# turbulencia/tlab

Measured on AMD Instinct MI355X. Metric: grid-point-updates/s per RK substep, higher is better.
Workload: dtype f64

## Files before the change

### tlab_amd/csrc/fftz.hip

```cpp
#include <hip/hip_runtime.h>

#include <cmath>
#include <cstdlib>
#include <stdexcept>
#include <string>
#include <vector>

#include "fftz.hpp"
#include "profile.hpp"

namespace tlab {

struct cd {
    double x, y;
};
__device__ __forceinline__ cd operator+(cd a, cd b) { return {a.x + b.x, a.y + b.y}; }
__device__ __forceinline__ cd operator-(cd a, cd b) { return {a.x - b.x, a.y - b.y}; }
__device__ __forceinline__ cd cmul(cd a, cd b) { return {a.x * b.x - a.y * b.y, a.x * b.y + a.y * b.x}; }
template <int SGN>
__device__ __forceinline__ cd mul_pm_i(cd a) {
    return SGN > 0 ? cd{-a.y, a.x} : cd{a.y, -a.x};
}

template <int SGN>
// ... 21 lines not shown
    v[1] = e1 + o1; v[5] = e1 - o1;
    v[2] = e2 + o2; v[6] = e2 - o2;
    v[3] = e3 + o3; v[7] = e3 - o3;
}

__device__ __forceinline__ int ilog2(int v) { return 31 - __builtin_clz(v); }

struct FftzArgs {
    const double2 *in;
    double2 *out;
    const double2 *tw;
    long long nlines;
    int n;
    int npass;
    int radix[8];
};

template <int R, int SGN, int T>
__device__ __forceinline__ void fftz_pass(const FftzArgs &a, int t, int j, int Ns, bool first, bool last, long long col, bool colok, cd *lds) {
    const int n = a.n, m = n / R;
    cd v[R];
    if (first) {
#pragma unroll
        for (int r = 0; r < R; ++r) {
            double2 w = make_double2(0.0, 0.0);
            if (colok) w = a.in[col + (long long)(j + r * m) * a.nlines];
            v[r] = {w.x, w.y};
        }
    } else {
#pragma unroll
        for (int r = 0; r < R; ++r) v[r] = lds[(j + r * m) * T + t];
    }
    const int lNs = ilog2(Ns), lR = ilog2(R), ln = ilog2(n);
    const int k0 = (j & (Ns - 1)) << (ln - lNs - lR);
#pragma unroll
    for (int r = 1; r < R; ++r) {
        const double2 w = a.tw[(k0 * r) & (n - 1)];
        v[r] = cmul(v[r], cd{w.x, SGN > 0 ? -w.y : w.y});
    }
    if (R == 8) dft8<SGN>(reinterpret_cast<cd(&)[8]>(v));
    else if (R == 4) dft4<SGN>(v[0], v[1 % R], v[2 % R], v[3 % R]);
    else dft2<SGN>(v[0], v[1 % R]);
    const int j0 = ((j >> lNs) << (lNs + lR)) + (j & (Ns - 1));
    if (!first) __syncthreads();
    if (last) {
        if (colok) {
#pragma unroll
            for (int r = 0; r < R; ++r) a.out[col + (long long)(j0 + r * Ns) * a.nlines] = make_double2(v[r].x, v[r].y);
        }
    } else {
#pragma unroll
        for (int r = 0; r < R; ++r) lds[(j0 + r * Ns) * T + t] = v[r];
        __syncthreads();
    }
}

template <int SGN, int T>
__global__ void __launch_bounds__(1024) k_fftz(FftzArgs a) {
    extern __shared__ double2 fz_lds[];
    cd *lds = reinterpret_cast<cd *>(fz_lds);
    const int t = threadIdx.x % T;
    const int jt = threadIdx.x / T;
    const long long col = (long long)blockIdx.x * T + t;
    const bool colok = col < a.nlines;
    int Ns = 1;
    for (int p = 0; p < a.npass; ++p) {
        const int R = a.radix[p];
        const bool first = p == 0, last = p == a.npass - 1;
        const int items = 8 / R;
        if (R == 8) {
            fftz_pass<8, SGN, T>(a, t, jt, Ns, first, last, col, colok, lds);
        } else {
            const int m8 = a.n / 8;
            if (R == 4) {
                cd keep[2][4];
                int j0s[2];
                for (int q = 0; q < 2; ++q) {
                    const int j = jt + q * m8, m = a.n / 4;
                    for (int r = 0; r < 4; ++r) {
                        if (first) {
                            double2 w = make_double2(0.0, 0.0);
                            if (colok) w = a.in[col + (long long)(j + r * m) * a.nlines];
                            keep[q][r] = {w.x, w.y};
                        } else {
                            keep[q][r] = lds[(j + r * m) * T + t];
                        }
                    }
                    const int k0 = (j & (Ns - 1)) * (a.n >> (ilog2(Ns) + 2));
                    for (int r = 1; r < 4; ++r) {
                        const double2 w = a.tw[(k0 * r) & (a.n - 1)];
                        keep[q][r] = cmul(keep[q][r], cd{w.x, SGN > 0 ? -w.y : w.y});
                    }
                    dft4<SGN>(keep[q][0], keep[q][1], keep[q][2], keep[q][3]);
                    j0s[q] = ((j >> ilog2(Ns)) << (ilog2(Ns) + 2)) + (j & (Ns - 1));
                }
                if (!first) __syncthreads();
                for (int q = 0; q < 2; ++q)
                    for (int r = 0; r < 4; ++r) {
                        if (last) {
                            if (colok) a.out[col + (long long)(j0s[q] + r * Ns) * a.nlines] = make_double2(keep[q][r].x, keep[q][r].y);
                        } else {
                            lds[(j0s[q] + r * Ns) * T + t] = keep[q][r];
                        }
                    }
                if (!last) __syncthreads();
            } else {
                cd keep[4][2];
                int j0s[4];
                for (int q = 0; q < 4; ++q) {
                    const int j = jt + q * m8, m = a.n / 2;
                    for (int r = 0; r < 2; ++r) {
                        if (first) {
                            double2 w = make_double2(0.0, 0.0);
                            if (colok) w = a.in[col + (long long)(j + r * m) * a.nlines];
                            keep[q][r] = {w.x, w.y};
                        } else {
                            keep[q][r] = lds[(j + r * m) * T + t];
                        }
                    }
                    const int k0 = (j & (Ns - 1)) * (a.n >> (ilog2(Ns) + 1));
                    const double2 w = a.tw[k0 & (a.n - 1)];
                    keep[q][1] = cmul(keep[q][1], cd{w.x, SGN > 0 ? -w.y : w.y});
                    dft2<SGN>(keep[q][0], keep[q][1]);
                    j0s[q] = ((j >> ilog2(Ns)) << (ilog2(Ns) + 1)) + (j & (Ns - 1));
                }
                if (!first) __syncthreads();
                for (int q = 0; q < 4; ++q)
                    for (int r = 0; r < 2; ++r) {
                        if (last) {
                            if (colok) a.out[col + (long long)(j0s[q] + r * Ns) * a.nlines] = make_double2(keep[q][r].x, keep[q][r].y);
                        } else {
                            lds[(j0s[q] + r * Ns) * T + t] = keep[q][r];
                        }
                    }
                if (!last) __syncthreads();
            }
            (void)items;
        }
        Ns *= R;
    }
}

struct FftxArgs {
    const double *in;
    double2 *out;
    const double2 *tw;
    long long nlines;
    int n, m;
    int npass;
    int radix[8];
    int tl, lines;
    const long long *kxoff;
    const int *kxw;
};

template <int R>
__device__ __forceinline__ void fftx_pass(const FftxArgs &a, const double2 *__restrict__ zin, bool ok, cd *lds, int jt, int Ns, bool first) {
    constexpr int Q = 8 / R;
    const int M = a.m, m = M / R;
    cd v[Q][R];
    int j0s[Q];
#pragma unroll
    for (int q = 0; q < Q; ++q) {
        const int j = jt + q * a.tl;
#pragma unroll
        for (int r = 0; r < R; ++r) {
            if (first) {
                double2 w = make_double2(0.0, 0.0);
// ... 59 lines not shown
        const cd B = {Zc.x, -Zc.y};
        const cd E = {0.5 * (A.x + B.x), 0.5 * (A.y + B.y)};
        const cd D = A - B;
        const cd O = {0.5 * D.y, -0.5 * D.x};
        const double2 w = a.tw[k];
        const cd T = cmul(cd{w.x, w.y}, O);
        out[k] = make_double2(E.x + T.x, E.y + T.y);
        if (k != M - k) out[M - k] = make_double2(E.x - T.x, -(E.y - T.y));
    }
}

struct FftxFinal {
    double *q, *h;
    double dte, kco;
    int scale, ny;
};

template <int R>
__device__ __forceinline__ void fftx_pass_inv(const FftxArgs &a, cd *lds, int jt, int Ns) {
    constexpr int Q = 8 / R;
    const int M = a.m, m = M / R;
    cd v[Q][R];
    int j0s[Q];
#pragma unroll
    for (int q = 0; q < Q; ++q) {
        const int j = jt + q * a.tl;
#pragma unroll
        for (int r = 0; r < R; ++r) v[q][r] = lds[j + r * m];
        const int k0 = (j & (Ns - 1)) << (ilog2(M) - ilog2(Ns) - ilog2(R));
#pragma unroll
// ... 2 lines not shown
            v[q][r] = cmul(v[q][r], cd{w.x, -w.y});
        }
        if (R == 8) dft8<+1>(reinterpret_cast<cd(&)[8]>(v[q]));
        else if (R == 4) dft4<+1>(v[q][0], v[q][1 % R], v[q][2 % R], v[q][3 % R]);
        else dft2<+1>(v[q][0], v[q][1 % R]);
        j0s[q] = ((j >> ilog2(Ns)) << (ilog2(Ns) + ilog2(R))) + (j & (Ns - 1));
    }
    __syncthreads();
#pragma unroll
    for (int q = 0; q < Q; ++q)
#pragma unroll
        for (int r = 0; r < R; ++r) lds[j0s[q] + r * Ns] = v[q][r];
    __syncthreads();
}

template <bool FINAL>
__global__ void __launch_bounds__(256) k_fftx_c2r(FftxArgs a, FftxFinal fin) {
    extern __shared__ double2 fx_lds[];
    const int jt = threadIdx.x & (a.tl - 1), ll = threadIdx.x >> ilog2(a.tl);
    const long long line = (long long)blockIdx.x * a.lines + ll;
    const bool ok = line < a.nlines;
    cd *lds = reinterpret_cast<cd *>(fx_lds) + (size_t)ll * a.m;
    const int M = a.m;
    if (ok) {
        const double2 *X = reinterpret_cast<const double2 *>(a.in) + line * (M + 1);
        const double2 *XP = reinterpret_cast<const double2 *>(a.in);
        for (int k = jt; k <= M / 2; k += a.tl) {
            double2 xa, xb;
            if (a.kxw != nullptr) { xa = XP[a.kxoff[k] + line * a.kxw[k]]; xb = XP[a.kxoff[M - k] + line * a.kxw[M - k]]; }
            else { xa = X[k]; xb = X[M - k]; }
            if (k == 0) { xa.y = 0.0; xb.y = 0.0; }
            const cd E = {xa.x + xb.x, xa.y - xb.y};
            const cd D = {xa.x - xb.x, xa.y + xb.y};
            const double2 w = a.tw[k];
            const cd O = cmul(D, cd{w.x, -w.y});
            if (k < M) lds[k % M] = {E.x - O.y, E.y + O.x};
            if (k != 0 && k != M - k) lds[M - k] = {E.x + O.y, -E.y + O.x};
        }
    }
    __syncthreads();
    int Ns = 1;
    for (int p = 0; p < a.npass; ++p) {
        const int R = a.radix[p];
        if (R == 8) fftx_pass_inv<8>(a, lds, jt, Ns);
        else if (R == 4) fftx_pass_inv<4>(a, lds, jt, Ns);
        else fftx_pass_inv<2>(a, lds, jt, Ns);
        Ns *= R;
    }
    if (!ok) return;
    if (!FINAL) {
        double2 *out = a.out + line * M;
        for (int j = jt; j < M; j += a.tl) out[j] = make_double2(lds[j].x, lds[j].y);
    } else {
        const int jy = a.nlines < (1LL << 31) ? (int)((unsigned)line % (unsigned)fin.ny) : (int)(line % fin.ny);
        const bool wall = jy == 0 || jy == fin.ny - 1;
        double2 *q2 = reinterpret_cast<double2 *>(fin.q) + line * M, *h2 = reinterpret_cast<double2 *>(fin.h) + line * M;
        for (int j = jt; j < M; j += a.tl) {
            const double2 hv0 = h2[j], qv = q2[j];
            double hx = hv0.x - lds[j].x, hy = hv0.y - lds[j].y;
            if (wall) { hx = 0.0; hy = 0.0; }
            q2[j] = make_double2(qv.x + fin.dte * hx, qv.y + fin.dte * hy);
            h2[j] = fin.scale ? make_double2(fin.kco * hx, fin.kco * hy) : make_double2(hx, hy);
        }
    }
}

bool FftxPlan::supported(int n) {
    if (n % 2 || n < 128 || n > 2048) return false;
    int m = n / 2;
    while (m % 8 == 0) m /= 8;
    return m == 1 || m == 2 || m == 4;
}

FftxPlan::FftxPlan(int n_, long long nlines_) : n(n_), nlines(nlines_) {
// ... 48 lines not shown
    const long double two_pi = 6.283185307179586476925286766559005768L;
    for (int k = 0; k < n; ++k) {
        tw[2 * k] = (double)cosl(two_pi * k / n);
        tw[2 * k + 1] = (double)(-sinl(two_pi * k / n));
    }
    if (hipMalloc((void **)&d_tw, tw.size() * sizeof(double)) != hipSuccess) throw std::runtime_error("FftzPlan: hipMalloc");
    if (hipMemcpy(d_tw, tw.data(), tw.size() * sizeof(double), hipMemcpyHostToDevice) != hipSuccess) throw std::runtime_error("FftzPlan: hipMemcpy");
}

FftzPlan::~FftzPlan() {
    if (d_tw) (void)hipFree(d_tw);
}

template <int T>
static void fftz_launch(int dir, const FftzArgs &a, hipStream_t st) {
    const unsigned grid = (unsigned)((a.nlines + T - 1) / T);
    const unsigned block = (unsigned)(T * a.n / 8);
    const size_t lds = (size_t)a.n * T * sizeof(double2);
    static bool attr_done = false;
    if (!attr_done) {
        (void)hipFuncSetAttribute(reinterpret_cast<const void *>(&k_fftz<-1, T>), hipFuncAttributeMaxDynamicSharedMemorySize, 160 * 1024);
        (void)hipFuncSetAttribute(reinterpret_cast<const void *>(&k_fftz<+1, T>), hipFuncAttributeMaxDynamicSharedMemorySize, 160 * 1024);
        (void)hipGetLastError();
        attr_done = true;
    }
    if (dir > 0) hipLaunchKernelGGL((k_fftz<-1, T>), dim3(grid), dim3(block), lds, st, a);
    else hipLaunchKernelGGL((k_fftz<+1, T>), dim3(grid), dim3(block), lds, st, a);
}

void FftzPlan::exec(int dir, const double *in, double *out, hipStream_t st) const {
    FftzArgs a{};
    a.in = reinterpret_cast<const double2 *>(in);
    a.out = reinterpret_cast<double2 *>(out);
    a.tw = reinterpret_cast<const double2 *>(d_tw);
    a.nlines = nlines; a.n = n; a.npass = (int)radix.size();
    for (size_t p = 0; p < radix.size(); ++p) a.radix[p] = radix[p];
    ProfScope ps("k_fftz", st, (double)nlines * n * 32.0);
    static const int t16 = [] { const char *e = getenv("TLAB_FFTZ_T"); return e ? atoi(e) : 8; }();
    if (n <= 512 && t16 == 16) fftz_launch<16>(dir, a, st);
    else if (n <= 1024) fftz_launch<8>(dir, a, st);
    else fftz_launch<4>(dir, a, st);
    if (hipGetLastError() != hipSuccess) throw std::runtime_error("k_fftz launch failed");
}

void FftxPlan::launch_inverse(const double *in, double *out, const double *q, const double *h, double dte, double kco, int scale, int ny,
                              hipStream_t st, const long long *kxoff, const int *kxw) const {
    FftxArgs a{};
    a.kxoff = kxoff; a.kxw = kxw;
    a.in = in;
    a.out = reinterpret_cast<double2 *>(out);
    a.tw = reinterpret_cast<const double2 *>(d_tw);
    a.nlines = nlines; a.n = n; a.m = n / 2; a.npass = (int)radix.size();
    for (size_t p = 0; p < radix.size(); ++p) a.radix[p] = radix[p];
    a.tl = a.m / 8;
    a.lines = a.tl >= 256 ? 1 : 256 / a.tl;
    const unsigned grid = (unsigned)((nlines + a.lines - 1) / a.lines);
    const size_t lds = (size_t)a.lines * a.m * sizeof(double2);
    FftxFinal f{const_cast<double *>(q), const_cast<double *>(h), dte, kco, scale, ny};
    if (q) {
        ProfScope ps("k_fftx_c2r<final>", st, (double)nlines * ((a.m + 1) * 16.0 + n * 32.0));
        hipLaunchKernelGGL(k_fftx_c2r<true>, dim3(grid), dim3((unsigned)(a.tl * a.lines)), lds, st, a, f);
    } else {
        ProfScope ps("k_fftx_c2r", st, (double)nlines * ((a.m + 1) * 16.0 + n * 8.0));
        hipLaunchKernelGGL(k_fftx_c2r<false>, dim3(grid), dim3((unsigned)(a.tl * a.lines)), lds, st, a, f);
    }
    if (hipGetLastError() != hipSuccess) throw std::runtime_error("k_fftx_c2r launch failed");
}

}
```

### tlab_amd/csrc/fftz.hpp

```cpp
#pragma once
#include <hip/hip_runtime.h>

#include <vector>

namespace tlab {

class FftzPlan {
public:
    static bool supported(int n);
    FftzPlan(int n, long long nlines);
    ~FftzPlan();
    FftzPlan(const FftzPlan &) = delete;
    FftzPlan &operator=(const FftzPlan &) = delete;
    void exec(int dir, const double *in, double *out, hipStream_t st) const;

private:
    int n;
    long long nlines;
    std::vector<int> radix;
    double *d_tw = nullptr;
};

class FftxPlan {
public:
    static bool supported(int n);
    FftxPlan(int n, long long nlines);
    ~FftxPlan();
    FftxPlan(const FftxPlan &) = delete;
    FftxPlan &operator=(const FftxPlan &) = delete;
    void exec(const double *in, double *out, hipStream_t st, const long long *kxoff = nullptr, const int *kxw = nullptr) const;
    void exec_inverse(const double *in, double *out, hipStream_t st, const long long *kxoff = nullptr, const int *kxw = nullptr) const {
        launch_inverse(in, out, nullptr, nullptr, 0.0, 0.0, 0, 0, st, kxoff, kxw);
    }
    void exec_inverse_final(const double *in, double *q, double *h, double dte, double kco, int scale, int ny, hipStream_t st,
                            const long long *kxoff = nullptr, const int *kxw = nullptr) const {
        launch_inverse(in, nullptr, q, h, dte, kco, scale, ny, st, kxoff, kxw);
    }

private:
    void launch_inverse(const double *in, double *out, const double *q, const double *h, double dte, double kco, int scale, int ny, hipStream_t st,
                        const long long *kxoff, const int *kxw) const;
    int n;
    long long nlines;
    std::vector<int> radix;
    double *d_tw = nullptr;
};

}
```

### tlab_amd/csrc/internal.hpp

```cpp
#pragma once
#include <hip/hip_runtime.h>

#include <string>
#include <vector>

#include "../../include/tlab_amd.h"

namespace tlab {
struct ScalarBounds;
}

hipStream_t tlab_current_stream();
void tlab_set_error(const std::string &s);
bool tlab_device_ready();
bool tlab_internal_partial_p1_fusable(int dir, tlab_fdm_plan_t g, int nx, int ny, int nz);
bool tlab_internal_partial_p1_fused(int dir, tlab_fdm_plan_t g, int nx, int ny, int nz, int ibc, const double *u, const double *ub,
                                    double scale, double *result, bool acc);
bool tlab_internal_partial_p1_sub(int dir, tlab_fdm_plan_t g, int nx, int ny, int nz, const double *u, double *result);
bool tlab_internal_neumann_final_ok(tlab_fdm_plan_t g, int nx, int ny, int nz);
bool tlab_internal_neumann_final(tlab_fdm_plan_t g, int nx, int ny, int nz, int ibc, double *h, double *q, double dte, double kco, int scale);
bool tlab_internal_gradient_final(int dir, tlab_fdm_plan_t g, int nx, int ny, int nz, const double *p, double *q, double *h, double dte,
                                  double kco, int scale, const double *pb = nullptr, const double *pt = nullptr);
bool tlab_internal_burgers_acc(int dir, tlab_fdm_plan_t g, int nx, int ny, int nz, int ibc, double nu, const double *s, const double *vel,
                               double *result);
// ... 8 lines not shown
extern "C" {
bool tlab_internal_anelastic();
int tlab_internal_anelastic_state(const double **rb, const double **rib, unsigned long *version);
bool tlab_internal_dealiasing();
void tlab_internal_dealiasing_forget(tlab_filter_t f);
}

int tlab_internal_deferred_flush();
int tlab_internal_deferred_take_error();

void tlab_internal_filter_1d(int dir, tlab_filter_t f, int nx, int ny, int nz, const double *u, double *result, hipStream_t st);

bool tlab_internal_poisson_has_own_x(tlab_poisson_plan_t P);
bool tlab_internal_poisson_can_v_final(tlab_poisson_plan_t P);
void tlab_internal_poisson_arm_v_final(tlab_poisson_plan_t P, double *q, double *h, double dte, double kco, int scale);

int tlab_internal_zslab_partial_z(tlab_zslab_plan_t P, int phase, int nx, int ny, const double *u, const double *const *u_halo, const double *ub,
                                  const double *const *ub_halo, double scale, double *head, double *tail, const double *tail_left,
                                  const double *head_right, double *result, int acc);
int tlab_internal_zslab_burgers_z_n(tlab_zslab_plan_t P, int phase, int nx, int ny, int nf, const double *nu, const double *const *s,
                                    const double *const *s_lo, const double *const *s_hi, const double *vel, double *head, double *tail,
                                    const double *tail_left, const double *head_right, double *const *result, int acc, const int *fin, double dte,
                                    double kco, int scale);
int tlab_internal_zslab_gradient_final_z(tlab_zslab_plan_t P, int nx, int ny, const double *p, const double *const *p_halo, const double *tail_left,
                                         const double *head_right, double *q, double *h, double dte, double kco, int scale);

long long tlab_internal_dns_points(tlab_dns_t d);
int tlab_internal_dns_nscal(tlab_dns_t d);
tlab::ScalarBounds *tlab_internal_dns_bounds(tlab_dns_t d);
bool tlab_internal_dns_has_flow_zones(tlab_dns_t d);
// ... 20 lines not shown
```

### tlab_amd/csrc/poisson.hip

```cpp
#include <hip/hip_runtime.h>

#include <type_traits>
#include <rocfft/rocfft.h>

#include <algorithm>
#include <cmath>
#include <cstdlib>
#include <memory>
#include <stdexcept>
#include <string>
#include <utility>
#include <vector>

#include "../../include/tlab_amd.h"
#include "internal.hpp"
#include "plan.hpp"
#include "fftz.hpp"
#include "poisson_host.hpp"
#include "int1_generic.hpp"
#include "profile.hpp"

namespace tlab {

struct Int1Dev {
// ... 1969 lines not shown
    int *d_hom_band = nullptr;
    int n_low = 0;
    DBuf low_f, low_p, low_dp;
    std::vector<int> sing_modes;
    int *d_sing = nullptr;
    unsigned char *d_skip = nullptr;
    DBuf s_lam, s_f, s_unit, s_bct, s_v0, s_v1, s_u0, s_u1, s_du0, s_du1, s_scr;
    DBuf dd_v1, dd_u1, dd_du1, dd_sp, dd_ones, dd_bcb;
    bool dd_ready = false;
    DBuf cst_dd;
    FftPlan fx_r2c, fx_c2r, fz_f, fz_b;
    FftPlan f2_fwd, f2_bwd;
    std::unique_ptr<FftzPlan> fz_own;
    std::unique_ptr<FftxPlan> fx_own;
    struct VFinal { double *q = nullptr, *h = nullptr; double dte = 0.0, kco = 0.0; int scale = 0; bool armed = false; } vfinal;
    void x_backward_dpdy(void *in, double *dpdy, hipStream_t st, const VFinal &f) {
        if (f.armed && fx_own) fx_own->exec_inverse_final(static_cast<const double *>(in), f.q, f.h, f.dte, f.kco, f.scale, ny, st);
        else fx_c2r.exec(in, dpdy, st);
    }
    void x_backward_p(void *in, double *p, hipStream_t st) {
        static const int own = [] { const char *e = getenv("TLAB_FFTX_C2R_OWN"); return e ? atoi(e) : -1; }();
        if (fx_own && (own == 1 || (own < 0 && nx >= 1024))) fx_own->exec_inverse(static_cast<const double *>(in), p, st);
        else fx_c2r.exec(in, p, st);
    }
    void x_forward(void *in, void *out, hipStream_t st) {
        if (fx_own) fx_own->exec(static_cast<const double *>(in), static_cast<double *>(out), st);
        else fx_r2c.exec(in, out, st);
    }
    struct KxMap { std::vector<long long> key; long long *off = nullptr; int *w = nullptr; };
    std::vector<KxMap> kxmaps;
// ... 582 lines not shown
        hipc(hipMalloc((void **)&P->d_skip, (size_t)nm), "hipMalloc");
        hipc(hipMemcpy(P->d_skip, skip.data(), (size_t)nm, hipMemcpyHostToDevice), "hipMemcpy");
        const int ns = (int)P->sing_modes.size();
        hipc(hipMalloc((void **)&P->d_sing, (ns + 1) * sizeof(int)), "hipMalloc");
        if (ns) hipc(hipMemcpy(P->d_sing, P->sing_modes.data(), ns * sizeof(int), hipMemcpyHostToDevice), "hipMemcpy");
        std::vector<double> slam(ns);
        for (int s = 0; s < ns; ++s) slam[s] = lam[P->sing_modes[s]];
        P->s_lam.upload(slam);
        const size_t n = ny;
        P->hom.alloc(5 * n * nm); P->der.alloc(3 * nm); P->cst.alloc(9 * nm);
        P->scratch.alloc(6 * n * nm);
        P->v0.alloc(2 * n * nm); P->u0.alloc(2 * n * nm); P->du0.alloc(2 * nm); P->bcs.alloc(4 * nm);
        P->helmholtz = helmholtz;
        if (!helmholtz) P->cwork.alloc((size_t)2 * P->nxh * ny * nz);
        if (nproc == 1 && nxl == 0) { P->g3[0] = gx; P->g3[1] = gy; P->g3[2] = gz; }
        P->s_f.alloc(2 * n * ns); P->s_bct.alloc(2 * ns); P->s_v0.alloc(2 * n * ns); P->s_v1.alloc(2 * n * ns);
        P->s_u0.alloc(2 * n * ns); P->s_u1.alloc(2 * n * ns); P->s_du0.alloc(2 * ns); P->s_du1.alloc(2 * ns); P->s_scr.alloc(5 * n * ns);
        if (!helmholtz) build_fft(*P);
        {
            const char *e = getenv("TLAB_FFT2D");
            if (!helmholtz && nzt > 1 && nproc == 1 && nxl == 0 && !P->fz_own && !(e && atoi(e) == 0)) {
                try {
                    build_fft_2d(*P);
                    P->use_2d = true;
                } catch (const std::exception &) {
                    P->use_2d = false;
                }
            }
        }
        create_side_stream(&P->side);
// ... 301 lines not shown
        tlab_set_error(e.what());                   \
        return TLAB_EINVAL;                         \
    }                                               \
    catch (const std::exception &e) {               \
        tlab_set_error(e.what());                   \
        return TLAB_EHIP;                           \
    }

int tlab_opr_poisson(tlab_poisson_plan_t P, int nx, int ny, int nz, int ibc, double *p, double *tmp1, double *tmp2,
                     const double *bcs_hb, const double *bcs_ht, double *dpdy) {
    POISSON_GUARD_BEGIN
    if (!P || !p || !tmp1 || !tmp2 || !bcs_hb || !bcs_ht) throw std::invalid_argument("tlab_opr_poisson: null argument");
    const tlab_poisson_plan::VFinal vf = P->vfinal;
    P->vfinal.armed = false;
    if (vf.armed && (!dpdy || !tlab_internal_poisson_can_v_final(P))) throw std::invalid_argument("tlab_opr_poisson: internal: the fused v update was requested from a plan that cannot do it");
    if (nx != P->nx || ny != P->ny || nz != P->nz) throw std::invalid_argument("tlab_opr_poisson: sizes do not match the plan");
    if (P->nproc != 1 || P->nxh != P->fx_nxh || P->fx_nz != P->nz)
        throw std::invalid_argument("tlab_opr_poisson: plan is a z-slab / kx-pencil plan; drive its stages with the transposes in between");
    if (ibc != TLAB_BCS_NN && ibc != TLAB_BCS_DD && !P->direct) {
        tlab_set_error("OPR_Poisson (factorized): BCS_NN and BCS_DD only, like the reference (opr_elliptic.f90:312-331)");
        return TLAB_EUNSUPPORTED;
    }
    if (ibc < TLAB_BCS_DD || ibc > TLAB_BCS_NN) throw std::invalid_argument("tlab_opr_poisson: bad ibc");
    if (p == tmp1 || p == tmp2 || tmp1 == tmp2 || dpdy == p || dpdy == tmp1 || dpdy == tmp2) throw std::invalid_argument("arrays must be distinct");
    if (P->direct) {
        hipStream_t st = tlab_current_stream();
        hipLaunchKernelGGL(k_set_wall_planes, dim3((unsigned)(((long long)nx * nz + 255) / 256)), dim3(256), 0, st, p, bcs_hb, bcs_ht, nx, ny, nz);
        if (nz > 1) {
            P->x_forward(p, tmp2, st);
            if (P->fz_own) P->fz_own->exec(1, tmp2, tmp1, st);
// ... 20 lines not shown
    if (P->use_2d) {
        P->f2_fwd.exec(p, tmp1, st);
    } else if (nz > 1) {
        P->x_forward(p, tmp2, st);
        if (P->fz_own) P->fz_own->exec(1, tmp2, tmp1, st);
        else P->fz_f.exec(tmp2, tmp1, st);
    } else {
        P->x_forward(p, tmp1, st);
    }
    if (ibc == TLAB_BCS_DD) poisson_dd_stage(P, tmp1, tmp1, tmp2, st);
    else poisson_ode_stage(P, tmp1, tmp1, tmp2, st);
    if (P->use_2d) {
        P->f2_bwd.exec(tmp1, p, st);
        if (dpdy) P->f2_bwd.exec(tmp2, dpdy, st);
    } else if (nz > 1) {
        if (P->fz_own) P->fz_own->exec(-1, tmp1, P->cwork.p, st);
        else P->fz_b.exec(tmp1, P->cwork.p, st);
        P->x_backward_p(P->cwork.p, p, st);
        if (dpdy) {
            if (P->fz_own) P->fz_own->exec(-1, tmp2, P->cwork.p, st);
            else P->fz_b.exec(tmp2, P->cwork.p, st);
            P->x_backward_dpdy(P->cwork.p, dpdy, st, vf);
        }
    } else {
        P->x_backward_p(tmp1, p, st);
        if (dpdy) P->x_backward_dpdy(tmp2, dpdy, st, vf);
    }
    POISSON_GUARD_END
}

int tlab_poisson_set_wall_planes(tlab_poisson_plan_t P, double *p, const double *bcs_hb, const double *bcs_ht) {
    POISSON_GUARD_BEGIN
    if (!P || !p || !bcs_hb || !bcs_ht) throw std::invalid_argument("null argument");
// ... 168 lines not shown
    } catch (const std::exception &e) {
        tlab_set_error(e.what());
        return TLAB_EHIP;
    }
}

}

bool tlab_internal_poisson_can_v_final(tlab_poisson_plan_t P) {
    static const bool on = [] { const char *e = getenv("TLAB_V_FINAL"); return !(e && atoi(e) == 0); }();
    return on && P && P->fx_own && !P->use_2d && !P->direct && !P->helmholtz && P->nproc == 1;
}
void tlab_internal_poisson_arm_v_final(tlab_poisson_plan_t P, double *q, double *h, double dte, double kco, int scale) {
    P->vfinal.q = q; P->vfinal.h = h; P->vfinal.dte = dte; P->vfinal.kco = kco; P->vfinal.scale = scale; P->vfinal.armed = true;
}
```

### tlab_amd/csrc/rhs.cpp

```cpp
#include "../../include/tlab_amd.h"

#include <hip/hip_runtime.h>

#include <algorithm>
#include <cmath>
#include <cstdlib>
#include <memory>
#include <string>
#include <functional>
#include <vector>

#include "driver_common.hpp"
#include "kernels.hpp"
#include "monitor.hpp"
#include "plan.hpp"

using namespace tlab;

struct tlab_dns {
    tlab_fdm_plan_t g[3];
    tlab_poisson_plan_t poisson;
    int nx, ny, nz, nscal;
    double visc;
    std::vector<double> schmidt;
// ... 486 lines not shown
    bool v_final = false;
    bool walls_dirichlet = true;
    for (int iq = 0; iq < 3; ++iq) walls_dirichlet = walls_dirichlet && d->bcs.flow_jmin[iq] == TLAB_DNS_BCS_DIRICHLET && d->bcs.flow_jmax[iq] == TLAB_DNS_BCS_DIRICHLET;
    auto ibc_y = [](int tmin, int tmax) { return (tmin == TLAB_DNS_BCS_NEUMANN ? 1 : 0) + (tmax == TLAB_DNS_BCS_NEUMANN ? 2 : 0); };
    bool any_neumann = false;
    for (int iq = 0; iq < 3; ++iq) any_neumann = any_neumann || ibc_y(d->bcs.flow_jmin[iq], d->bcs.flow_jmax[iq]) != 0;
    for (int is = 0; is < d->nscal; ++is) any_neumann = any_neumann || ibc_y(d->bcs.scal_jmin[is], d->bcs.scal_jmax[is]) != 0;
    const bool neu_fast = any_neumann && tail_update && d->fuse && !literal && nz > 1 && !d->pfilter[0] && !d->pfilter[1] && !d->pfilter[2] && !any_surface &&
                          tlab_internal_poisson_can_v_final(d->poisson) && tlab_internal_neumann_final_ok(gy, nx, ny, nz) &&
                          tlab_internal_partial_p1_fusable(1, gx, nx, ny, nz) && tlab_internal_partial_p1_fusable(3, gz, nx, ny, nz);
    if (tail_update && d->fuse && !literal && !d->pfilter[0] && !d->pfilter[1] && !d->pfilter[2] && (walls_dirichlet || neu_fast) &&
        tlab_internal_poisson_can_v_final(d->poisson)) {
        tlab_internal_poisson_arm_v_final(d->poisson, q[1], hq[1], dte, kco, scale_tendencies);
        v_final = true;
    }
    ok(tlab_opr_poisson(d->poisson, nx, ny, nz, TLAB_BCS_NN, tmp1, tmp2, tmp4, d->bcs_hb, d->bcs_ht, tmp3), "OPR_Poisson");
    if (d->pfilter[0] || d->pfilter[1] || d->pfilter[2]) {
        ok(tlab_opr_filter(nx, ny, nz, d->pfilter[0], d->pfilter[1], d->pfilter[2], d->pfilter_rep, tmp1, tmp4), "OPR_FILTER(p)");
        ok(tlab_opr_filter(nx, ny, nz, d->pfilter[0], d->pfilter[1], d->pfilter[2], d->pfilter_rep, tmp3, tmp4), "OPR_FILTER(dpdy)");
    }
    if (scal_neumann_planes && !neu_fast) throw Fail(TLAB_EINVAL, "internal: Neumann scalars were finished without their wall planes");
    if (neu_fast) {
        const char *npe = getenv("TLAB_NEUMANN_PLANES");
        const bool neu_planes = !(npe && atoi(npe) == 0);
        for (int iq = 0; iq < 3; iq += 2) {
            const int dir = iq == 0 ? 1 : 3;
            tlab_fdm_plan_t gd = iq == 0 ? gx : gz;
            const int ibc = ibc_y(d->bcs.flow_jmin[iq], d->bcs.flow_jmax[iq]);
            bool done;
            if (ibc == 0) done = tlab_internal_gradient_final(dir, gd, nx, ny, nz, tmp1, q[iq], hq[iq], dte, kco, scale_tendencies);
            else if (neu_planes && neumann_weights(d, ibc)) {
                const tlab_dns::NeuW &W = d->neuw[ibc];
                const size_t np = (size_t)nx * nz;
                if (!d->wall_planes) hk(hipMalloc((void **)&d->wall_planes, 6 * np * sizeof(double)), "hipMalloc");
                double *Hb = d->wall_planes, *Ht = Hb + np, *Pb = Ht + np, *Pt = Pb + np, *Db = Pt + np, *Dt = Db + np;
                hk(launch_wall_weighted(hq[iq], tmp1, W.w, W.w + W.K, W.K, Hb, Ht, Pb, Pt, nx, ny, nz, st), "wall planes");
                ok(tlab_opr_partial(dir, gd, TLAB_OPR_P1, nx, 1, nz, 0, Pb, Db, nullptr), "OPR_Partial (wall plane)");
                ok(tlab_opr_partial(dir, gd, TLAB_OPR_P1, nx, 1, nz, 0, Pt, Dt, nullptr), "OPR_Partial (wall plane)");
                hk(launch_sub2(Hb, Hb, Db, (long long)np, st), "wall planes");
                hk(launch_sub2(Ht, Ht, Dt, (long long)np, st), "wall planes");
// ... 20 lines not shown
        }
        for (int is = 0; is < d->nscal && finish_scal && scal_neumann_planes; ++is) {
            const int ibc = ibc_y(d->bcs.scal_jmin[is], d->bcs.scal_jmax[is]);
            if (ibc == 0) continue;
            const tlab_dns::NeuW &W = d->neuw[ibc];
            const size_t np = (size_t)nx * nz;
            if (!d->wall_planes) hk(hipMalloc((void **)&d->wall_planes, 6 * np * sizeof(double)), "hipMalloc");
            double *Sb = d->wall_planes, *St = Sb + np;
            hk(launch_wall_weighted(hs[is], nullptr, W.w, W.w + W.K, W.K, Sb, St, nullptr, nullptr, nx, ny, nz, st), "wall planes");
            hk(launch_wall_fix(s[is], hs[is], (ibc & 1) ? Sb : nullptr, (ibc & 2) ? St : nullptr, dte, kco, scale_tendencies, nx, ny, nz, st, clip_of(d, is)),
               "wall planes");
        }
        return;
    }
    bool grad_final = false, grad_sub = false;
    if (tail_update && d->fuse && nz > 1 && !literal) {
        bool dirichlet = true;
        for (int iq = 0; iq < 3; ++iq) dirichlet = dirichlet && d->bcs.flow_jmin[iq] == TLAB_DNS_BCS_DIRICHLET && d->bcs.flow_jmax[iq] == TLAB_DNS_BCS_DIRICHLET;
        if (dirichlet && tlab_internal_partial_p1_fusable(1, gx, nx, ny, nz) && tlab_internal_partial_p1_fusable(3, gz, nx, ny, nz)) {
            const bool okx = tlab_internal_gradient_final(1, gx, nx, ny, nz, tmp1, q[0], hq[0], dte, kco, scale_tendencies);
            const bool okz = okx && tlab_internal_gradient_final(3, gz, nx, ny, nz, tmp1, q[2], hq[2], dte, kco, scale_tendencies);
            if (okx != okz) throw Fail(TLAB_EINVAL, "internal: inconsistent fused gradient path");
            grad_final = okx;
        }
    }
    if (stag) {
        ok(tlab_opr_partial(3, gz, TLAB_OPR_P0_INT_PV, nx, ny, nz, B0, tmp3, tmp5, nullptr), "OPR_Partial_Z(P0_INT_PV)");
        ok(tlab_opr_partial(1, gx, TLAB_OPR_P0_INT_PV, nx, ny, nz, B0, tmp5, tmp3, nullptr), "OPR_Partial_X(P0_INT_PV)");
        ok(tlab_opr_partial(3, gz, TLAB_OPR_P1_INT_PV, nx, ny, nz, B0, tmp1, tmp5, nullptr), "OPR_Partial_Z(P1_INT_PV)");
        ok(tlab_opr_partial(1, gx, TLAB_OPR_P0_INT_PV, nx, ny, nz, B0, tmp5, tmp4, nullptr), "OPR_Partial_X(P0_INT_PV)");
        ok(tlab_opr_partial(3, gz, TLAB_OPR_P0_INT_PV, nx, ny, nz, B0, tmp1, tmp5, nullptr), "OPR_Partial_Z(P0_INT_PV)");
// ... 606 lines not shown
```

Before: 8.527 billion.

## Compute x/z pressure gradients spectrally inside the Poisson inverse transforms

Instead of inverse-transforming pressure and then applying finite-difference x and z derivatives, the periodic-uniform case multiplies by the modified wavenumbers inside the inverse FFTs. A dual z-FFT kernel emits both the plain and the ik_z-scaled spectra in one launch, and the c2r x-transform fuses the ik_x or Jacobian scaling together with the u and w RK updates. This removes the separate gradient-partial passes and their global memory traffic for u and w. In exchange it adds an extra inverse x-FFT, a larger dual kernel, and a dependence on the modified-wavenumber symbol matching the compact FD scheme.

```diff
diff --git a/tlab_amd/csrc/fftz.hip b/tlab_amd/csrc/fftz.hip
--- a/tlab_amd/csrc/fftz.hip
+++ b/tlab_amd/csrc/fftz.hip
@@ -59,10 +59,13 @@
     int n;
     int npass;
     int radix[8];
+    double2 *out2;
+    const double *kp;
 };
 
-template <int R, int SGN, int T>
-__device__ __forceinline__ void fftz_pass(const FftzArgs &a, int t, int j, int Ns, bool first, bool last, long long col, bool colok, cd *lds) {
+template <int R, int SGN, int T, int DUAL = 0>
+__device__ __forceinline__ void fftz_pass(const FftzArgs &a, int t, int j, int Ns, bool first, bool last, long long col, bool colok, cd *lds,
+                                          bool ik = false, double2 *out = nullptr) {
     const int n = a.n, m = n / R;
     cd v[R];
     if (first) {
@@ -70,6 +73,10 @@
         for (int r = 0; r < R; ++r) {
             double2 w = make_double2(0.0, 0.0);
             if (colok) w = a.in[col + (long long)(j + r * m) * a.nlines];
+            if (DUAL) {
+                const double kp = a.kp[j + r * m], b = ik ? kp : 0.0, c = ik ? 0.0 : 1.0;
+                w = make_double2(c * w.x - b * w.y, c * w.y + b * w.x);
+            }
             v[r] = {w.x, w.y};
         }
     } else {
@@ -90,8 +97,9 @@
     if (!first) __syncthreads();
     if (last) {
         if (colok) {
-#pragma unroll
-            for (int r = 0; r < R; ++r) a.out[col + (long long)(j0 + r * Ns) * a.nlines] = make_double2(v[r].x, v[r].y);
+            double2 *o = DUAL ? out : a.out;
+#pragma unroll
+            for (int r = 0; r < R; ++r) o[col + (long long)(j0 + r * Ns) * a.nlines] = make_double2(v[r].x, v[r].y);
         }
     } else {
 #pragma unroll
@@ -100,21 +108,24 @@
     }
 }
 
-template <int SGN, int T>
+template <int SGN, int T, int DUAL>
 __global__ void __launch_bounds__(1024) k_fftz(FftzArgs a) {
     extern __shared__ double2 fz_lds[];
     cd *lds = reinterpret_cast<cd *>(fz_lds);
     const int t = threadIdx.x % T;
     const int jt = threadIdx.x / T;
-    const long long col = (long long)blockIdx.x * T + t;
+    constexpr int TL = DUAL == 1 ? T / 2 : T;
+    const bool ik = DUAL == 2 || (DUAL == 1 && t >= TL);
+    const long long col = (long long)blockIdx.x * TL + (DUAL == 1 ? t % TL : t);
     const bool colok = col < a.nlines;
+    double2 *const outp = (DUAL == 1 && ik) ? a.out2 : a.out;
     int Ns = 1;
     for (int p = 0; p < a.npass; ++p) {
         const int R = a.radix[p];
         const bool first = p == 0, last = p == a.npass - 1;
         const int items = 8 / R;
         if (R == 8) {
-            fftz_pass<8, SGN, T>(a, t, jt, Ns, first, last, col, colok, lds);
+            fftz_pass<8, SGN, T, DUAL>(a, t, jt, Ns, first, last, col, colok, lds, ik, outp);
         } else {
             const int m8 = a.n / 8;
             if (R == 4) {
@@ -143,7 +154,7 @@
                 for (int q = 0; q < 2; ++q)
                     for (int r = 0; r < 4; ++r) {
                         if (last) {
-                            if (colok) a.out[col + (long long)(j0s[q] + r * Ns) * a.nlines] = make_double2(keep[q][r].x, keep[q][r].y);
+                            if (colok) (DUAL ? outp : a.out)[col + (long long)(j0s[q] + r * Ns) * a.nlines] = make_double2(keep[q][r].x, keep[q][r].y);
                         } else {
                             lds[(j0s[q] + r * Ns) * T + t] = keep[q][r];
                         }
@@ -173,7 +184,7 @@
                 for (int q = 0; q < 4; ++q)
                     for (int r = 0; r < 2; ++r) {
                         if (last) {
-                            if (colok) a.out[col + (long long)(j0s[q] + r * Ns) * a.nlines] = make_double2(keep[q][r].x, keep[q][r].y);
+                            if (colok) (DUAL ? outp : a.out)[col + (long long)(j0s[q] + r * Ns) * a.nlines] = make_double2(keep[q][r].x, keep[q][r].y);
                         } else {
                             lds[(j0s[q] + r * Ns) * T + t] = keep[q][r];
                         }
@@ -197,6 +208,7 @@
     int tl, lines;
     const long long *kxoff;
     const int *kxw;
+    const double *kp;
 };
 
 template <int R>
@@ -286,6 +298,7 @@
     double *q, *h;
     double dte, kco;
     int scale, ny;
+    const double *rj, *rl;
 };
 
 template <int R>
@@ -318,8 +331,9 @@
     __syncthreads();
 }
 
-template <bool FINAL>
+template <bool FINAL, int GRAD>
 __global__ void __launch_bounds__(256) k_fftx_c2r(FftxArgs a, FftxFinal fin) {
+    constexpr bool IK = GRAD == 1;
     extern __shared__ double2 fx_lds[];
     const int jt = threadIdx.x & (a.tl - 1), ll = threadIdx.x >> ilog2(a.tl);
     const long long line = (long long)blockIdx.x * a.lines + ll;
@@ -334,6 +348,11 @@
             if (a.kxw != nullptr) { xa = XP[a.kxoff[k] + line * a.kxw[k]]; xb = XP[a.kxoff[M - k] + line * a.kxw[M - k]]; }
             else { xa = X[k]; xb = X[M - k]; }
             if (k == 0) { xa.y = 0.0; xb.y = 0.0; }
+            if (IK) {
+                const double ka = a.kp[k], kb = a.kp[M - k];
+                xa = make_double2(-ka * xa.y, ka * xa.x);
+                xb = make_double2(-kb * xb.y, kb * xb.x);
+            }
             const cd E = {xa.x + xb.x, xa.y - xb.y};
             const cd D = {xa.x - xb.x, xa.y + xb.y};
             const double2 w = a.tw[k];
@@ -359,9 +378,14 @@
         const int jy = a.nlines < (1LL << 31) ? (int)((unsigned)line % (unsigned)fin.ny) : (int)(line % fin.ny);
         const bool wall = jy == 0 || jy == fin.ny - 1;
         double2 *q2 = reinterpret_cast<double2 *>(fin.q) + line * M, *h2 = reinterpret_cast<double2 *>(fin.h) + line * M;
+        const double rl = GRAD == 2 ? fin.rl[a.nlines < (1LL << 31) ? (long long)((unsigned)line / (unsigned)fin.ny) : line / fin.ny] : 1.0;
+        const double2 *rj2 = reinterpret_cast<const double2 *>(fin.rj);
         for (int j = jt; j < M; j += a.tl) {
             const double2 hv0 = h2[j], qv = q2[j];
-            double hx = hv0.x - lds[j].x, hy = hv0.y - lds[j].y;
+            double gx = lds[j].x, gy = lds[j].y;
+            if (GRAD == 1) { const double2 r = rj2[j]; gx *= r.x; gy *= r.y; }
+            if (GRAD == 2) { gx *= rl; gy *= rl; }
+            double hx = hv0.x - gx, hy = hv0.y - gy;
             if (wall) { hx = 0.0; hy = 0.0; }
             q2[j] = make_double2(qv.x + fin.dte * hx, qv.y + fin.dte * hy);
             h2[j] = fin.scale ? make_double2(fin.kco * hx, fin.kco * hy) : make_double2(hx, hy);
@@ -440,39 +464,54 @@
 
 template <int T>
 static void fftz_launch(int dir, const FftzArgs &a, hipStream_t st) {
-    const unsigned grid = (unsigned)((a.nlines + T - 1) / T);
+    const int tl = a.out2 ? T / 2 : T;
+    const unsigned grid = (unsigned)((a.nlines + tl - 1) / tl);
     const unsigned block = (unsigned)(T * a.n / 8);
     const size_t lds = (size_t)a.n * T * sizeof(double2);
     static bool attr_done = false;
     if (!attr_done) {
-        (void)hipFuncSetAttribute(reinterpret_cast<const void *>(&k_fftz<-1, T>), hipFuncAttributeMaxDynamicSharedMemorySize, 160 * 1024);
-        (void)hipFuncSetAttribute(reinterpret_cast<const void *>(&k_fftz<+1, T>), hipFuncAttributeMaxDynamicSharedMemorySize, 160 * 1024);
+        (void)hipFuncSetAttribute(reinterpret_cast<const void *>(&k_fftz<-1, T, 0>), hipFuncAttributeMaxDynamicSharedMemorySize, 160 * 1024);
+        (void)hipFuncSetAttribute(reinterpret_cast<const void *>(&k_fftz<+1, T, 0>), hipFuncAttributeMaxDynamicSharedMemorySize, 160 * 1024);
+        (void)hipFuncSetAttribute(reinterpret_cast<const void *>(&k_fftz<+1, T, 2>), hipFuncAttributeMaxDynamicSharedMemorySize, 160 * 1024);
+        if constexpr (T == 16) (void)hipFuncSetAttribute(reinterpret_cast<const void *>(&k_fftz<+1, T, 1>), hipFuncAttributeMaxDynamicSharedMemorySize, 160 * 1024);
         (void)hipGetLastError();
         attr_done = true;
     }
-    if (dir > 0) hipLaunchKernelGGL((k_fftz<-1, T>), dim3(grid), dim3(block), lds, st, a);
-    else hipLaunchKernelGGL((k_fftz<+1, T>), dim3(grid), dim3(block), lds, st, a);
-}
-
-void FftzPlan::exec(int dir, const double *in, double *out, hipStream_t st) const {
+    if constexpr (T == 16) {
+        if (a.out2) { hipLaunchKernelGGL((k_fftz<+1, T, 1>), dim3(grid), dim3(block), lds, st, a); return; }
+    }
+    if (a.kp) hipLaunchKernelGGL((k_fftz<+1, T, 2>), dim3(grid), dim3(block), lds, st, a);
+    else if (dir > 0) hipLaunchKernelGGL((k_fftz<-1, T, 0>), dim3(grid), dim3(block), lds, st, a);
+    else hipLaunchKernelGGL((k_fftz<+1, T, 0>), dim3(grid), dim3(block), lds, st, a);
+}
+
+bool FftzPlan::dual_supported(int n) { return supported(n) && n <= 512; }
+
+void FftzPlan::exec(int dir, const double *in, double *out, hipStream_t st, double *out2, const double *kp) const {
+    if ((out2 && !kp) || (kp && dir > 0) || (out2 && (out2 == out || in == out || !dual_supported(n)))) throw std::invalid_argument("FftzPlan: bad dual transform");
     FftzArgs a{};
     a.in = reinterpret_cast<const double2 *>(in);
     a.out = reinterpret_cast<double2 *>(out);
+    a.out2 = reinterpret_cast<double2 *>(out2);
+    a.kp = kp;
     a.tw = reinterpret_cast<const double2 *>(d_tw);
     a.nlines = nlines; a.n = n; a.npass = (int)radix.size();
     for (size_t p = 0; p < radix.size(); ++p) a.radix[p] = radix[p];
-    ProfScope ps("k_fftz", st, (double)nlines * n * 32.0);
+    ProfScope ps(out2 ? "k_fftz<dual>" : kp ? "k_fftz<ik>" : "k_fftz", st, (double)nlines * n * (out2 ? 48.0 : 32.0));
     static const int t16 = [] { const char *e = getenv("TLAB_FFTZ_T"); return e ? atoi(e) : 8; }();
-    if (n <= 512 && t16 == 16) fftz_launch<16>(dir, a, st);
+    if (out2) fftz_launch<16>(dir, a, st);
+    else if (n <= 512 && t16 == 16) fftz_launch<16>(dir, a, st);
     else if (n <= 1024) fftz_launch<8>(dir, a, st);
     else fftz_launch<4>(dir, a, st);
     if (hipGetLastError() != hipSuccess) throw std::runtime_error("k_fftz launch failed");
 }
 
 void FftxPlan::launch_inverse(const double *in, double *out, const double *q, const double *h, double dte, double kco, int scale, int ny,
-                              hipStream_t st, const long long *kxoff, const int *kxw) const {
+                              hipStream_t st, const long long *kxoff, const int *kxw, const double *kp, const double *rj, const double *rl) const {
+    if ((kp || rj || rl) && !q) throw std::invalid_argument("FftxPlan: the gradient forms exist in the final form only");
+    if ((kp != nullptr) != (rj != nullptr) || (kp && rl)) throw std::invalid_argument("FftxPlan: bad gradient form");
     FftxArgs a{};
-    a.kxoff = kxoff; a.kxw = kxw;
+    a.kxoff = kxoff; a.kxw = kxw; a.kp = kp;
     a.in = in;
     a.out = reinterpret_cast<double2 *>(out);
     a.tw = reinterpret_cast<const double2 *>(d_tw);
@@ -482,13 +521,19 @@
     a.lines = a.tl >= 256 ? 1 : 256 / a.tl;
     const unsigned grid = (unsigned)((nlines + a.lines - 1) / a.lines);
     const size_t lds = (size_t)a.lines * a.m * sizeof(double2);
-    FftxFinal f{const_cast<double *>(q), const_cast<double *>(h), dte, kco, scale, ny};
-    if (q) {
+    FftxFinal f{const_cast<double *>(q), const_cast<double *>(h), dte, kco, scale, ny, rj, rl};
+    if (q && kp) {
+        ProfScope ps("k_fftx_c2r<final,ik>", st, (double)nlines * ((a.m + 1) * 16.0 + n * 32.0));
+        hipLaunchKernelGGL((k_fftx_c2r<true, 1>), dim3(grid), dim3((unsigned)(a.tl * a.lines)), lds, st, a, f);
+    } else if (q && rl) {
+        ProfScope ps("k_fftx_c2r<final,z>", st, (double)nlines * ((a.m + 1) * 16.0 + n * 32.0));
+        hipLaunchKernelGGL((k_fftx_c2r<true, 2>), dim3(grid), dim3((unsigned)(a.tl * a.lines)), lds, st, a, f);
+    } else if (q) {
         ProfScope ps("k_fftx_c2r<final>", st, (double)nlines * ((a.m + 1) * 16.0 + n * 32.0));
-        hipLaunchKernelGGL(k_fftx_c2r<true>, dim3(grid), dim3((unsigned)(a.tl * a.lines)), lds, st, a, f);
+        hipLaunchKernelGGL((k_fftx_c2r<true, 0>), dim3(grid), dim3((unsigned)(a.tl * a.lines)), lds, st, a, f);
     } else {
         ProfScope ps("k_fftx_c2r", st, (double)nlines * ((a.m + 1) * 16.0 + n * 8.0));
-        hipLaunchKernelGGL(k_fftx_c2r<false>, dim3(grid), dim3((unsigned)(a.tl * a.lines)), lds, st, a, f);
+        hipLaunchKernelGGL((k_fftx_c2r<false, 0>), dim3(grid), dim3((unsigned)(a.tl * a.lines)), lds, st, a, f);
     }
     if (hipGetLastError() != hipSuccess) throw std::runtime_error("k_fftx_c2r launch failed");
 }
diff --git a/tlab_amd/csrc/fftz.hpp b/tlab_amd/csrc/fftz.hpp
--- a/tlab_amd/csrc/fftz.hpp
+++ b/tlab_amd/csrc/fftz.hpp
@@ -12,7 +12,8 @@
     ~FftzPlan();
     FftzPlan(const FftzPlan &) = delete;
     FftzPlan &operator=(const FftzPlan &) = delete;
-    void exec(int dir, const double *in, double *out, hipStream_t st) const;
+    static bool dual_supported(int n);
+    void exec(int dir, const double *in, double *out, hipStream_t st, double *out2 = nullptr, const double *kp = nullptr) const;
 
 private:
     int n;
@@ -30,16 +31,17 @@
     FftxPlan &operator=(const FftxPlan &) = delete;
     void exec(const double *in, double *out, hipStream_t st, const long long *kxoff = nullptr, const int *kxw = nullptr) const;
     void exec_inverse(const double *in, double *out, hipStream_t st, const long long *kxoff = nullptr, const int *kxw = nullptr) const {
-        launch_inverse(in, out, nullptr, nullptr, 0.0, 0.0, 0, 0, st, kxoff, kxw);
+        launch_inverse(in, out, nullptr, nullptr, 0.0, 0.0, 0, 0, st, kxoff, kxw, nullptr, nullptr, nullptr);
     }
     void exec_inverse_final(const double *in, double *q, double *h, double dte, double kco, int scale, int ny, hipStream_t st,
-                            const long long *kxoff = nullptr, const int *kxw = nullptr) const {
-        launch_inverse(in, nullptr, q, h, dte, kco, scale, ny, st, kxoff, kxw);
+                            const long long *kxoff = nullptr, const int *kxw = nullptr, const double *kp = nullptr, const double *rj = nullptr,
+                            const double *rl = nullptr) const {
+        launch_inverse(in, nullptr, q, h, dte, kco, scale, ny, st, kxoff, kxw, kp, rj, rl);
     }
 
 private:
     void launch_inverse(const double *in, double *out, const double *q, const double *h, double dte, double kco, int scale, int ny, hipStream_t st,
-                        const long long *kxoff, const int *kxw) const;
+                        const long long *kxoff, const int *kxw, const double *kp, const double *rj, const double *rl) const;
     int n;
     long long nlines;
     std::vector<int> radix;
diff --git a/tlab_amd/csrc/internal.hpp b/tlab_amd/csrc/internal.hpp
--- a/tlab_amd/csrc/internal.hpp
+++ b/tlab_amd/csrc/internal.hpp
@@ -46,6 +46,8 @@
 bool tlab_internal_poisson_has_own_x(tlab_poisson_plan_t P);
 bool tlab_internal_poisson_can_v_final(tlab_poisson_plan_t P);
 void tlab_internal_poisson_arm_v_final(tlab_poisson_plan_t P, double *q, double *h, double dte, double kco, int scale);
+bool tlab_internal_poisson_can_uw_final(tlab_poisson_plan_t P, tlab_fdm_plan_t gx, tlab_fdm_plan_t gz);
+void tlab_internal_poisson_arm_uw_final(tlab_poisson_plan_t P, double *qu, double *hu, double *qw, double *hw, double dte, double kco, int scale);
 
 int tlab_internal_zslab_partial_z(tlab_zslab_plan_t P, int phase, int nx, int ny, const double *u, const double *const *u_halo, const double *ub,
                                   const double *const *ub_halo, double scale, double *head, double *tail, const double *tail_left,
diff --git a/tlab_amd/csrc/poisson.hip b/tlab_amd/csrc/poisson.hip
--- a/tlab_amd/csrc/poisson.hip
+++ b/tlab_amd/csrc/poisson.hip
@@ -2007,6 +2007,9 @@
     std::unique_ptr<FftzPlan> fz_own;
     std::unique_ptr<FftxPlan> fx_own;
     struct VFinal { double *q = nullptr, *h = nullptr; double dte = 0.0, kco = 0.0; int scale = 0; bool armed = false; } vfinal;
+    struct UWFinal { double *qu = nullptr, *hu = nullptr, *qw = nullptr, *hw = nullptr; double dte = 0.0, kco = 0.0; int scale = 0; bool armed = false; } uwfinal;
+    DBuf uw_kx, uw_kz;
+    DBuf uw_rjx, uw_rjz;
     void x_backward_dpdy(void *in, double *dpdy, hipStream_t st, const VFinal &f) {
         if (f.armed && fx_own) fx_own->exec_inverse_final(static_cast<const double *>(in), f.q, f.h, f.dte, f.kco, f.scale, ny, st);
         else fx_c2r.exec(in, dpdy, st);
@@ -2619,6 +2622,18 @@
         P->helmholtz = helmholtz;
         if (!helmholtz) P->cwork.alloc((size_t)2 * P->nxh * ny * nz);
         if (nproc == 1 && nxl == 0) { P->g3[0] = gx; P->g3[1] = gy; P->g3[2] = gz; }
+        auto symbol_ok = [](const tlab::FdmTables &t) {
+            return t.periodic && t.uniform && !t.stagger && t.der1.ndl == 3 && !t.der1.direct && t.n % 2 == 0 && (int)t.jac.size() >= t.n && t.jac[0] > 0.0;
+        };
+        if (!helmholtz && nproc == 1 && nxl == 0 && nzt > 1 && symbol_ok(gx->t) && symbol_ok(gz->t)) {
+            std::vector<double> kx(gx->t.der1.mwn.begin(), gx->t.der1.mwn.begin() + nx / 2 + 1), kz(gz->t.der1.mwn);
+            kx[nx / 2] = 0.0; kz[nzt / 2] = 0.0;
+            P->uw_kx.upload(kx); P->uw_kz.upload(kz);
+            std::vector<double> rx(nx), rz(nzt);
+            for (int i = 0; i < nx; ++i) rx[i] = gx->t.jac[0] / gx->t.jac[i];
+            for (int k = 0; k < nzt; ++k) rz[k] = gz->t.jac[0] / gz->t.jac[k];
+            P->uw_rjx.upload(rx); P->uw_rjz.upload(rz);
+        }
         P->s_f.alloc(2 * n * ns); P->s_bct.alloc(2 * ns); P->s_v0.alloc(2 * n * ns); P->s_v1.alloc(2 * n * ns);
         P->s_u0.alloc(2 * n * ns); P->s_u1.alloc(2 * n * ns); P->s_du0.alloc(2 * ns); P->s_du1.alloc(2 * ns); P->s_scr.alloc(5 * n * ns);
         if (!helmholtz) build_fft(*P);
@@ -2950,6 +2965,10 @@
     const tlab_poisson_plan::VFinal vf = P->vfinal;
     P->vfinal.armed = false;
     if (vf.armed && (!dpdy || !tlab_internal_poisson_can_v_final(P))) throw std::invalid_argument("tlab_opr_poisson: internal: the fused v update was requested from a plan that cannot do it");
+    const tlab_poisson_plan::UWFinal uw = P->uwfinal;
+    P->uwfinal.armed = false;
+    if (uw.armed && (!vf.armed || ibc != TLAB_BCS_NN || !tlab_internal_poisson_can_uw_final(P, P->g3[0], P->g3[2])))
+        throw std::invalid_argument("tlab_opr_poisson: internal: the fused u, w updates were requested from a plan that cannot do them");
     if (nx != P->nx || ny != P->ny || nz != P->nz) throw std::invalid_argument("tlab_opr_poisson: sizes do not match the plan");
     if (P->nproc != 1 || P->nxh != P->fx_nxh || P->fx_nz != P->nz)
         throw std::invalid_argument("tlab_opr_poisson: plan is a z-slab / kx-pencil plan; drive its stages with the transposes in between");
@@ -3000,9 +3019,17 @@
         P->f2_bwd.exec(tmp1, p, st);
         if (dpdy) P->f2_bwd.exec(tmp2, dpdy, st);
     } else if (nz > 1) {
-        if (P->fz_own) P->fz_own->exec(-1, tmp1, P->cwork.p, st);
-        else P->fz_b.exec(tmp1, P->cwork.p, st);
-        P->x_backward_p(P->cwork.p, p, st);
+        if (uw.armed) {
+            static const bool dual = [] { const char *e = getenv("TLAB_FFTZ_DUAL"); return !(e && atoi(e) == 0); }();
+            if (dual) P->fz_own->exec(-1, tmp1, P->cwork.p, st, tmp1, P->uw_kz.p);
+            else { P->fz_own->exec(-1, tmp1, P->cwork.p, st); P->fz_own->exec(-1, tmp1, tmp1, st, nullptr, P->uw_kz.p); }
+            P->fx_own->exec_inverse_final(P->cwork.p, uw.qu, uw.hu, uw.dte, uw.kco, uw.scale, ny, st, nullptr, nullptr, P->uw_kx.p, P->uw_rjx.p);
+            P->fx_own->exec_inverse_final(tmp1, uw.qw, uw.hw, uw.dte, uw.kco, uw.scale, ny, st, nullptr, nullptr, nullptr, nullptr, P->uw_rjz.p);
+        } else {
+            if (P->fz_own) P->fz_own->exec(-1, tmp1, P->cwork.p, st);
+            else P->fz_b.exec(tmp1, P->cwork.p, st);
+            P->x_backward_p(P->cwork.p, p, st);
+        }
         if (dpdy) {
             if (P->fz_own) P->fz_own->exec(-1, tmp2, P->cwork.p, st);
             else P->fz_b.exec(tmp2, P->cwork.p, st);
@@ -3201,3 +3228,10 @@
 void tlab_internal_poisson_arm_v_final(tlab_poisson_plan_t P, double *q, double *h, double dte, double kco, int scale) {
     P->vfinal.q = q; P->vfinal.h = h; P->vfinal.dte = dte; P->vfinal.kco = kco; P->vfinal.scale = scale; P->vfinal.armed = true;
 }
+bool tlab_internal_poisson_can_uw_final(tlab_poisson_plan_t P, tlab_fdm_plan_t gx, tlab_fdm_plan_t gz) {
+    return tlab_internal_poisson_can_v_final(P) && P->fz_own && P->nzt > 1 && FftzPlan::dual_supported(P->nzt) && P->uw_kx.p && P->uw_kz.p && P->uw_rjx.p && P->uw_rjz.p && gx && gz && gx == P->g3[0] && gz == P->g3[2];
+}
+void tlab_internal_poisson_arm_uw_final(tlab_poisson_plan_t P, double *qu, double *hu, double *qw, double *hw, double dte, double kco, int scale) {
+    P->uwfinal.qu = qu; P->uwfinal.hu = hu; P->uwfinal.qw = qw; P->uwfinal.hw = hw;
+    P->uwfinal.dte = dte; P->uwfinal.kco = kco; P->uwfinal.scale = scale; P->uwfinal.armed = true;
+}
diff --git a/tlab_amd/csrc/rhs.cpp b/tlab_amd/csrc/rhs.cpp
--- a/tlab_amd/csrc/rhs.cpp
+++ b/tlab_amd/csrc/rhs.cpp
@@ -524,6 +524,14 @@
         tlab_internal_poisson_arm_v_final(d->poisson, q[1], hq[1], dte, kco, scale_tendencies);
         v_final = true;
     }
+    bool uw_final = false;
+    {
+        const char *sge = getenv("TLAB_SPECTRAL_GRADIENT");
+        if (v_final && walls_dirichlet && nz > 1 && !(sge && atoi(sge) == 0) && tlab_internal_poisson_can_uw_final(d->poisson, gx, gz)) {
+            tlab_internal_poisson_arm_uw_final(d->poisson, q[0], hq[0], q[2], hq[2], dte, kco, scale_tendencies);
+            uw_final = true;
+        }
+    }
     ok(tlab_opr_poisson(d->poisson, nx, ny, nz, TLAB_BCS_NN, tmp1, tmp2, tmp4, d->bcs_hb, d->bcs_ht, tmp3), "OPR_Poisson");
     if (d->pfilter[0] || d->pfilter[1] || d->pfilter[2]) {
         ok(tlab_opr_filter(nx, ny, nz, d->pfilter[0], d->pfilter[1], d->pfilter[2], d->pfilter_rep, tmp1, tmp4), "OPR_FILTER(p)");
@@ -533,7 +541,7 @@
     if (neu_fast) {
         const char *npe = getenv("TLAB_NEUMANN_PLANES");
         const bool neu_planes = !(npe && atoi(npe) == 0);
-        for (int iq = 0; iq < 3; iq += 2) {
+        for (int iq = 0; iq < 3 && !uw_final; iq += 2) {
             const int dir = iq == 0 ? 1 : 3;
             tlab_fdm_plan_t gd = iq == 0 ? gx : gz;
             const int ibc = ibc_y(d->bcs.flow_jmin[iq], d->bcs.flow_jmax[iq]);
@@ -584,7 +592,9 @@
         return;
     }
     bool grad_final = false, grad_sub = false;
-    if (tail_update && d->fuse && nz > 1 && !literal) {
+    if (uw_final) {
+        grad_final = true;
+    } else if (tail_update && d->fuse && nz > 1 && !literal) {
         bool dirichlet = true;
         for (int iq = 0; iq < 3; ++iq) dirichlet = dirichlet && d->bcs.flow_jmin[iq] == TLAB_DNS_BCS_DIRICHLET && d->bcs.flow_jmax[iq] == TLAB_DNS_BCS_DIRICHLET;
         if (dirichlet && tlab_internal_partial_p1_fusable(1, gx, nx, ny, nz) && tlab_internal_partial_p1_fusable(3, gz, nx, ny, nz)) {
```

Result: slower. 8.417 billion (-1.3%).
